# ChrisTho23/DrakeGPT

Hardware: NVIDIA B200
Metric: train_tokens_per_sec_TransformerLM_scaled (higher is better)
Workload: dtype bf16

## Files before the change

### drakegpt_b200/csrc/attn_tc.cu

```cuda
#include <cuda.h>

#include "common.cuh"
#include "ptx.cuh"

namespace dgpt {

using namespace ptx;

int make_tmap_bf16_2d(CUtensorMap* map, const void* base, int64_t inner, int64_t outer, int64_t ld, int box_outer);

static constexpr int HD = 64;
static constexpr int QT = 128;
static constexpr float kLog2e = 1.4426950408889634f;

struct AttnTcP {
  void *o, *dq, *dk, *dv;
  const void *o_in, *d_o;
  float* lse;
  int64_t o_rs, dq_rs, dk_rs, dv_rs, do_rs;
  int B, NH, T;
  float scale, inv_keep;
  uint32_t thr, site;
  uint64_t seed;
  const uint64_t* seed_dev;
};

__device__ __forceinline__ uint32_t pack_bf16(float a, float b) {
  __nv_bfloat162 v = __floats2bfloat162_rn(a, b);
  return *reinterpret_cast<uint32_t*>(&v);
}

__device__ __forceinline__ void store_row32_sw128(uint8_t* tile_base, int row, int c0, const float (&v)[32]) {
  uint8_t* blk = tile_base + (c0 >> 6) * 16384 + row * 128;
  const int chunk0 = (c0 & 63) >> 3;
#pragma unroll
  for (int j = 0; j < 4; ++j) {
    uint4 w;
    w.x = pack_bf16(v[8 * j], v[8 * j + 1]);
    w.y = pack_bf16(v[8 * j + 2], v[8 * j + 3]);
    w.z = pack_bf16(v[8 * j + 4], v[8 * j + 5]);
    w.w = pack_bf16(v[8 * j + 6], v[8 * j + 7]);
    *reinterpret_cast<uint4*>(blk + (((chunk0 + j) ^ (row & 7)) << 4)) = w;
  }
}

static constexpr int kFwd2Threads = 320;
static constexpr int kFwd2QK = 49152;
static constexpr int kFwd2Smem = 2 * kFwd2QK + 2 * 32768 + 256 + 1024;
static constexpr int kWHeavy = 5, kWLight = 2;

struct FwdSched {
  int nheavy, nlight;
  unsigned long long* probe;
};

__global__ void __launch_bounds__(kFwd2Threads, 1)
attn_fwd_tc2_kernel(const __grid_constant__ CUtensorMap map_q32, const __grid_constant__ CUtensorMap map_k,
                    const __grid_constant__ CUtensorMap map_v, AttnTcP p, FwdSched sc) {
  extern __shared__ uint8_t smem_raw[];
  uint8_t* smem = reinterpret_cast<uint8_t*>((reinterpret_cast<uintptr_t>(smem_raw) + 1023) & ~(uintptr_t)1023);
  uint8_t* sQK = smem;
  uint8_t* sV = smem + 2 * kFwd2QK;
  uint64_t* bars = reinterpret_cast<uint64_t*>(sV + 2 * 32768);
  uint64_t *qk_full = bars, *qk_empty = bars + 2, *v_full = bars + 4, *v_empty = bars + 6, *s_full = bars + 8,
           *p_full = bars + 10, *o_full = bars + 12, *slot_free = bars + 14;
  uint32_t* tmem_slot = reinterpret_cast<uint32_t*>(bars + 16);

  clock_probe_begin(sc.probe);
  const int warp = threadIdx.x >> 5, lane = threadIdx.x & 31;
  const int ntile = p.T / QT;

  const int G = gridDim.x, c = blockIdx.x;
  const int hq = sc.nheavy / G, hr = sc.nheavy % G;
  const int nh_c = hq + (c < hr ? 1 : 0);
  const int U = (kWHeavy * sc.nheavy + kWLight * sc.nlight + G - 1) / G;
  const int cap_hi = max(0, (U - kWHeavy * (hq + 1)) / kWLight), cap_lo = max(0, (U - kWHeavy * hq) / kWLight);
  const int cap_total = hr * cap_hi + (G - hr) * cap_lo;
  const int l_start = c < hr ? c * cap_hi : hr * cap_hi + (c - hr) * cap_lo;
  const int l0 = min(sc.nlight, l_start), l1 = min(sc.nlight, l_start + (c < hr ? cap_hi : cap_lo));
  const int n_extra = cap_total < sc.nlight ? (sc.nlight - cap_total - c + G - 1) / G : 0;
  const int n_items = nh_c + (l1 - l0) + max(0, n_extra);
  auto item = [&](int n, int& bh, int& qt) {
    if (n < nh_c) {
      const int hi = c + n * G;
      bh = hi; qt = ntile - 1;
    } else {
      const int m = n - nh_c;
      const int li = m < l1 - l0 ? l0 + m : cap_total + c + (m - (l1 - l0)) * G;
      bh = li; qt = 0;
    }
  };

  if (threadIdx.x == 0) {
    prefetch_tensormap(&map_q32);
    prefetch_tensormap(&map_k);
    prefetch_tensormap(&map_v);
    for (int g = 0; g < 2; ++g) {
      mbar_init(&qk_full[g], 1);
      mbar_init(&qk_empty[g], 1);
      mbar_init(&v_full[g], 1);
      mbar_init(&v_empty[g], 1);
      mbar_init(&s_full[g], 1);
      mbar_init(&p_full[g], 4);
      mbar_init(&o_full[g], 1);
      mbar_init(&slot_free[g], 4);
    }
    fence_barrier_init();
  }
  if (warp == 9) tmem_alloc<512>(tmem_slot);
  tc_fence_before();
  __syncthreads();
  tc_fence_after();
  const uint32_t tmem = *tmem_slot;
  pdl_grid_sync();

  if (warp == 8) {
    for (int n = 0; n < n_items; ++n) {
      const int g = n & 1, k = n >> 1;
      int bh, qt;
      item(n, bh, qt);
      const int nkv = qt + 1, b = bh / p.NH, h = bh % p.NH, row0 = b * p.T;
      uint8_t* q_s = sQK + g * kFwd2QK;
      uint8_t* v_s = sV + g * 32768;
      mbar_wait(&qk_empty[g], (k & 1) ^ 1);
      if (elect_one()) {
        mbar_expect_tx(&qk_full[g], 16384 * (1 + nkv));
        for (int qb = 0; qb < 4; ++qb)
          tma_load_2d(q_s + qb * 4096, &map_q32, &qk_full[g], h * HD, row0 + qt * QT + (g ? 3 - qb : qb) * 32);
        for (int j = 0; j < nkv; ++j) tma_load_2d(q_s + 16384 * (1 + j), &map_k, &qk_full[g], h * HD, row0 + j * QT);
      }
      __syncwarp();
      mbar_wait(&v_empty[g], (k & 1) ^ 1);
      if (elect_one()) {
        mbar_expect_tx(&v_full[g], 16384 * nkv);
        for (int kb = 0; kb < 2 * nkv; ++kb) tma_load_2d(v_s + kb * 8192, &map_v, &v_full[g], h * HD, row0 + kb * 64);
      }
      __syncwarp();
    }
  } else if (warp == 9) {
    constexpr uint32_t idesc_s = make_idesc_bf16(128, 128, 0, 0);
    constexpr uint32_t idesc_o = make_idesc_bf16(128, 64, 0, 1);
    int next_s = 0, next_pv = 0;
    while (next_pv < n_items) {
      bool progressed = false;
      if (next_s < n_items) {
        const int g = next_s & 1, k = next_s >> 1;
        if (mbar_test(&qk_full[g], k & 1) && mbar_test(&slot_free[g], (k & 1) ^ 1)) {
          tc_fence_after();
          int bh, qt;
          item(next_s, bh, qt);
          const int nkv = qt + 1;
          const uint64_t dq0 = make_smem_desc_sw128(smem_u32(sQK + g * kFwd2QK), 16, 1024);
          const uint64_t dk0 = make_smem_desc_sw128(smem_u32(sQK + g * kFwd2QK + 16384), 16, 1024);
          if (elect_one()) {
            for (int j = 0; j < nkv; ++j) {
#pragma unroll
              for (int kk = 0; kk < 4; ++kk)
                tc_mma_bf16(tmem + g * 256 + j * 128, dq0 + (uint64_t)(kk * 2), dk0 + (uint64_t)(j * 1024 + kk * 2), idesc_s, kk > 0);
            }
            tc_commit(&s_full[g]);
            tc_commit(&qk_empty[g]);
          }
          __syncwarp();
          ++next_s;
          progressed = true;
        }
      }
      if (next_pv < next_s) {
        const int g = next_pv & 1, k = next_pv >> 1;
        if (mbar_test(&p_full[g], k & 1) && mbar_test(&v_full[g], k & 1)) {
          tc_fence_after();
          int bh, qt;
          item(next_pv, bh, qt);
          const int nkv = qt + 1;
          const uint64_t dv0 = make_smem_desc_sw128(smem_u32(sV + g * 32768), 8192, 1024);
          if (elect_one()) {
            for (int kb = 0; kb < 2 * nkv; ++kb) {
#pragma unroll
              for (int kk = 0; kk < 4; ++kk)
                tc_mma_bf16_ts(tmem + g * 256 + nkv * 64, tmem + g * 256 + kb * 32 + kk * 8, dv0 + (uint64_t)(kb * 512 + kk * 128),
                               idesc_o, (kb | kk) > 0);
            }
            tc_commit(&o_full[g]);
            tc_commit(&v_empty[g]);
          }
          __syncwarp();
          ++next_pv;
          progressed = true;
        }
      }
      if (!progressed) __nanosleep(32);
    }
  } else {
    const int g = warp >> 2;
    const int quad = warp & 3;
    const int rblk = g ? 3 - quad : quad;
    const int row = rblk * 32 + lane;
    const uint32_t taddr = tmem + (uint32_t)(g * 256) + ((uint32_t)(quad * 32) << 16);
    uint64_t seed = p.seed;
    if (p.thr && p.seed_dev) seed += *p.seed_dev;
    const float sc2 = p.scale * kLog2e;
    for (int n = g; n < n_items; n += 2) {
      const int k = n >> 1;
      int bh, qt;
      item(n, bh, qt);
      const int nkv = qt + 1, b = bh / p.NH, h = bh % p.NH, row0 = b * p.T;
      const int qg = qt * QT + row;
      const int ncols = nkv * QT;
#define FTS(i) do { if (sc.probe && blockIdx.x == 0 && warp == 0 && lane == 0 && k < 3) sc.probe[4 + k * 8 + (i)] = (unsigned long long)clock64(); } while (0)
      FTS(0);
      mbar_wait(&s_full[g], k & 1);
      FTS(1);
      tc_fence_after();
      const int qg_max = qt * QT + rblk * 32 + 31, qg_min = qt * QT + rblk * 32;
      float mx = -INFINITY;
      for (int cc = 0; cc < ncols && cc <= qg_max; cc += 32) {
        uint32_t r[32];
        tmem_ld32(taddr + cc, r);
        tmem_ld_wait();
        if (cc + 31 <= qg_min) {
#pragma unroll
          for (int j = 0; j < 32; ++j) mx = fmaxf(mx, __uint_as_float(r[j]));
        } else {
#pragma unroll
          for (int j = 0; j < 32; ++j)
            if (cc + j <= qg) mx = fmaxf(mx, __uint_as_float(r[j]));
        }
      }
      FTS(2);
      const float msc = mx * sc2;
      float sum = 0.f;
      const uint64_t base = (((uint64_t)b * p.NH + h) * p.T + qg) * (uint64_t)p.T;
      for (int cc = 0; cc < ncols; cc += 32) {
        float e[32];
        if (cc > qg_max) {
#pragma unroll
          for (int j = 0; j < 32; ++j) e[j] = 0.f;
        } else {
          uint32_t r[32];
          tmem_ld32(taddr + cc, r);
          tmem_ld_wait();
          if (cc + 31 <= qg_min) {
#pragma unroll
            for (int j = 0; j < 32; ++j) {
              const float v = exp2f(__uint_as_float(r[j]) * sc2 - msc);
              sum += v;
              e[j] = v;
            }
          } else {
#pragma unroll
            for (int j = 0; j < 32; ++j) {
              const float v = (cc + j <= qg) ? exp2f(__uint_as_float(r[j]) * sc2 - msc) : 0.f;
              sum += v;
              e[j] = v;
            }
          }
          if (p.thr) {
            const DropGroup dg = dropout_group(seed, p.site, (base + cc) >> 5);
#pragma unroll
            for (int j = 0; j < 32; ++j)
              if (dropout_word(dg, j) < p.thr) e[j] = 0.f;
          }
        }
        uint32_t pk[16];
#pragma unroll
        for (int j = 0; j < 16; ++j) pk[j] = pack_bf16(e[2 * j], e[2 * j + 1]);
        tmem_st16(taddr + (cc >> 1), pk);
      }
      if (p.lse) p.lse[((int64_t)b * p.NH + h) * p.T + qg] = mx * p.scale + logf(sum);
      tmem_st_wait();
      tc_fence_before();
      __syncwarp();
      if (lane == 0) mbar_arrive(&p_full[g]);
      FTS(3);
      mbar_wait(&o_full[g], k & 1);
      FTS(4);
      tc_fence_after();
      const float oscale = p.inv_keep / sum;
      __nv_bfloat16* orow = reinterpret_cast<__nv_bfloat16*>(p.o) + (int64_t)(row0 + qg) * p.o_rs + h * HD;
#pragma unroll
      for (int cc = 0; cc < HD; cc += 32) {
        uint32_t r[32];
        tmem_ld32(taddr + nkv * 64 + cc, r);
        tmem_ld_wait();
#pragma unroll
        for (int j = 0; j < 4; ++j) {
          uint4 w;
          w.x = pack_bf16(__uint_as_float(r[8 * j]) * oscale, __uint_as_float(r[8 * j + 1]) * oscale);
          w.y = pack_bf16(__uint_as_float(r[8 * j + 2]) * oscale, __uint_as_float(r[8 * j + 3]) * oscale);
          w.z = pack_bf16(__uint_as_float(r[8 * j + 4]) * oscale, __uint_as_float(r[8 * j + 5]) * oscale);
          w.w = pack_bf16(__uint_as_float(r[8 * j + 6]) * oscale, __uint_as_float(r[8 * j + 7]) * oscale);
          *reinterpret_cast<uint4*>(orow + cc + 8 * j) = w;
        }
      }
      tc_fence_before();
      __syncwarp();
      if (lane == 0) mbar_arrive(&slot_free[g]);
      FTS(5);
    }
  }
  tc_fence_before();
  __syncthreads();
  if (warp == 9) {
    tc_fence_after();
    tmem_dealloc<512>(tmem);
  }
  clock_probe_end(sc.probe);
}

#ifdef DGPT_ATTN_TS
__device__ long long g_attn_ts[64];
#endif
static constexpr int kBwdThreads = 64 + 256;
static constexpr int kBwdSmem = 8 * 16384 + 2 * 32768 + 16384 + 2048 + 1024 + 128;

template <bool DIAG, bool DROP>
__device__ __forceinline__ void bwd_chunk_math(const AttnTcP& p, uint32_t lane_addr_st, uint32_t lane_addr_dp, int row, int k0,
                                               float sc, float lse2, float Dq, uint64_t seed, uint64_t base,
                                               float (&pd)[32], float (&ds)[32]) {
  uint32_t st[32], dp[32];
  tmem_ld32(lane_addr_st + k0, st);
  tmem_ld32(lane_addr_dp + k0, dp);
  tmem_ld_wait();
  DropGroup g = {0u, 0u};
  if (DROP) g = dropout_group(seed, p.site, (base + k0) >> 5);
#pragma unroll
  for (int t = 0; t < 32; ++t) {
    float pv = exp2f(__uint_as_float(st[t]) * sc - lse2);
    if (DIAG) pv = (k0 + t) <= row ? pv : 0.f;
    float dpv = __uint_as_float(dp[t]);
    float pdv = pv;
    if (DROP) {
      const bool keep = dropout_word(g, t) >= p.thr;
      dpv = keep ? dpv * p.inv_keep : 0.f;
      pdv = keep ? pv * p.inv_keep : 0.f;
    }
    pd[t] = pdv;
    ds[t] = pv * (dpv - Dq) * p.scale;
  }
}

template <bool DROP>
__global__ void __launch_bounds__(kBwdThreads, 1)
attn_bwd_tc_kernel(const __grid_constant__ CUtensorMap map_q, const __grid_constant__ CUtensorMap map_k,
                   const __grid_constant__ CUtensorMap map_v, const __grid_constant__ CUtensorMap map_do,
                   const __grid_constant__ CUtensorMap map_o, const __grid_constant__ CUtensorMap map_dq,
                   const __grid_constant__ CUtensorMap map_dk, const __grid_constant__ CUtensorMap map_dv, AttnTcP p) {
  extern __shared__ __align__(1024) uint8_t smem[];
  uint8_t* sQ = smem;
  uint8_t* sK = smem + 2 * 16384;
  uint8_t* sV = smem + 4 * 16384;
  uint8_t* sG = smem + 6 * 16384;
  uint8_t* sPd = smem + 8 * 16384;
  uint8_t* sDs = sPd + 32768;
  uint8_t* sSt = sDs + 32768;
  float* lse_s = reinterpret_cast<float*>(sSt + 16384);
  float* D_s = lse_s + 256;
  uint64_t* bars = reinterpret_cast<uint64_t*>(D_s + 256);
  uint64_t *ld_a = bars, *st_full = bars + 1, *ps_full = bars + 2, *drained = bars + 3, *acc_done = bars + 4;
  uint64_t *ld_b = bars + 5, *ld_c = bars + 6;
  uint64_t* acc_free = bars + 7;
  uint32_t* tmem_slot = reinterpret_cast<uint32_t*>(bars + 8);

  const int warp = threadIdx.x >> 5, lane = threadIdx.x & 31;
#ifdef DGPT_ATTN_TS
#define BTS(i) do { if (blockIdx.x == 0 && blockIdx.y == (gridDim.y / 2) && warp == 2 && lane == 0) g_attn_ts[i] = clock64(); } while (0)
#else
#define BTS(i) do { } while (0)
#endif
  BTS(0);
  const int h = blockIdx.x, b = blockIdx.y;
  const int ntile = p.T / QT;
  const int npair = ntile == 1 ? 1 : 3;
  const int row0 = b * p.T;

  if (threadIdx.x == 0) {
    prefetch_tensormap(&map_q);
    prefetch_tensormap(&map_k);
    prefetch_tensormap(&map_v);
    prefetch_tensormap(&map_do);
    prefetch_tensormap(&map_o);
    mbar_init(ld_a, 1);
    mbar_init(ld_b, 1);
    mbar_init(ld_c, 1);
    mbar_init(st_full, 1);
    mbar_init(ps_full, 8);
    mbar_init(drained, 8);
    mbar_init(acc_done, 1);
    mbar_init(acc_free, 1);
    fence_barrier_init();
  }
  if (warp == 0) {
    __syncwarp();
    pdl_grid_sync();
    if (elect_one()) {
      mbar_expect_tx(ld_a, 16384 * 5);
      tma_load_2d(sG, &map_do, ld_a, h * HD, row0);
      tma_load_2d(sPd, &map_o, ld_a, h * HD, row0);
      tma_load_2d(sQ, &map_q, ld_a, h * HD, row0);
      tma_load_2d(sK, &map_k, ld_a, h * HD, row0);
      tma_load_2d(sV, &map_v, ld_a, h * HD, row0);
      if (ntile > 1) {
        mbar_expect_tx(ld_b, 16384 * 3);
        tma_load_2d(sG + 16384, &map_do, ld_b, h * HD, row0 + QT);
        tma_load_2d(sSt, &map_o, ld_b, h * HD, row0 + QT);
        tma_load_2d(sQ + 16384, &map_q, ld_b, h * HD, row0 + QT);
        mbar_expect_tx(ld_c, 16384 * 2);
        tma_load_2d(sK + 16384, &map_k, ld_c, h * HD, row0 + QT);
        tma_load_2d(sV + 16384, &map_v, ld_c, h * HD, row0 + QT);
      }
    }
  }
  if (warp == 1) tmem_alloc<512>(tmem_slot);
  tc_fence_before();
  __syncthreads();
  tc_fence_after();
  const uint32_t tmem = *tmem_slot;
  constexpr uint32_t TM_ST = 0, TM_DP = 128, TM_DV = 256, TM_DK = 320, TM_DQ = 384;
  if (warp != 0) pdl_grid_sync();

  if (warp == 0) {
  } else if (warp == 1) {
    constexpr uint32_t id_kk = make_idesc_bf16(128, 128, 0, 0);
    constexpr uint32_t id_kmn = make_idesc_bf16(128, 64, 0, 1);
    constexpr uint32_t id_mnmn = make_idesc_bf16(128, 64, 1, 1);
    mbar_wait(ld_a, 0);
    tc_fence_after();
    const uint64_t kQ = make_smem_desc_sw128(smem_u32(sQ), 16, 1024), kK = make_smem_desc_sw128(smem_u32(sK), 16, 1024);
    const uint64_t kV = make_smem_desc_sw128(smem_u32(sV), 16, 1024), kG = make_smem_desc_sw128(smem_u32(sG), 16, 1024);
    const uint64_t kDs = make_smem_desc_sw128(smem_u32(sDs), 16, 1024);
    const uint64_t mQ = make_smem_desc_sw128(smem_u32(sQ), 8192, 1024), mK = make_smem_desc_sw128(smem_u32(sK), 8192, 1024);
    const uint64_t mG = make_smem_desc_sw128(smem_u32(sG), 8192, 1024);
    const uint64_t mPd = make_smem_desc_sw128(smem_u32(sPd), 16384, 1024), mDs = make_smem_desc_sw128(smem_u32(sDs), 16384, 1024);
    auto issue_s_dp = [&](int pr) {
      const int i = pr == 0 ? 0 : 1, j = pr == 2 ? 1 : 0;
      if (elect_one()) {
#pragma unroll
        for (int k = 0; k < 4; ++k)
          tc_mma_bf16(tmem + TM_ST, kQ + (uint64_t)(i * 1024 + k * 2), kK + (uint64_t)(j * 1024 + k * 2), id_kk, k > 0);
#pragma unroll
        for (int k = 0; k < 4; ++k)
          tc_mma_bf16(tmem + TM_DP, kG + (uint64_t)(i * 1024 + k * 2), kV + (uint64_t)(j * 1024 + k * 2), id_kk, k > 0);
        tc_commit(st_full);
      }
      __syncwarp();
    };
    issue_s_dp(0);
    for (int pr = 0; pr < npair; ++pr) {
      const int i = pr == 0 ? 0 : 1, j = pr == 2 ? 1 : 0;
      mbar_wait(ps_full, pr & 1);
      if (pr + 1 < npair) {
        mbar_wait(pr + 1 == 1 ? ld_b : ld_c, 0);
        tc_fence_after();
        issue_s_dp(pr + 1);
      }
      if (pr > 0) mbar_wait(drained, (pr - 1) & 1);
      tc_fence_after();
      const uint32_t acc_vk = (pr == 1) ? 1u : 0u;
      const uint32_t acc_q = (pr == 2) ? 1u : 0u;
      if (elect_one()) {
#pragma unroll
        for (int k = 0; k < 8; ++k)
          tc_mma_bf16(tmem + TM_DV, mPd + (uint64_t)(k * 128), mG + (uint64_t)(i * 1024 + k * 128), id_mnmn, acc_vk | (k > 0));
#pragma unroll
        for (int k = 0; k < 8; ++k)
          tc_mma_bf16(tmem + TM_DK, mDs + (uint64_t)(k * 128), mQ + (uint64_t)(i * 1024 + k * 128), id_mnmn, acc_vk | (k > 0));
#pragma unroll
        for (int k = 0; k < 8; ++k)
          tc_mma_bf16(tmem + TM_DQ, kDs + (uint64_t)((k >> 2) * 1024 + (k & 3) * 2), mK + (uint64_t)(j * 1024 + k * 128), id_kmn,
                      acc_q | (k > 0));
        tc_commit(acc_free);
        if (pr == npair - 1) tc_commit(acc_done);
      }
      __syncwarp();
    }
  } else {
    const int cw = warp - 2;
    const int quad = warp & 3;
    const int half = cw >> 2;
    const int rowl = quad * 32 + lane;
    const int ct = threadIdx.x - 64;
    const uint32_t lane_addr = tmem + ((uint32_t)(quad * 32) << 16);
    uint64_t seed = p.seed;
    if (DROP && p.seed_dev) seed += *p.seed_dev;
    if (ct < p.T) lse_s[ct] = p.lse[((int64_t)b * p.NH + h) * p.T + ct] * kLog2e;
    auto compute_D = [&](int tl, const uint8_t* o_tile) {
      if (ct < QT) {
        const int r = ct;
        const uint8_t* gr = sG + tl * 16384 + r * 128;
        const uint8_t* orow = o_tile + r * 128;
        float acc = 0.f;
#pragma unroll
        for (int c = 0; c < 8; ++c) {
          const int off = (c ^ (r & 7)) << 4;
          const uint4 g = *reinterpret_cast<const uint4*>(gr + off), o = *reinterpret_cast<const uint4*>(orow + off);
          const uint32_t gw[4] = {g.x, g.y, g.z, g.w}, ow[4] = {o.x, o.y, o.z, o.w};
#pragma unroll
          for (int t = 0; t < 4; ++t) {
            const float2 gf = __bfloat1622float2(*reinterpret_cast<const __nv_bfloat162*>(&gw[t]));
            const float2 of = __bfloat1622float2(*reinterpret_cast<const __nv_bfloat162*>(&ow[t]));
            acc = fmaf(gf.x, of.x, acc);
            acc = fmaf(gf.y, of.y, acc);
          }
        }
        D_s[tl * QT + r] = acc;
      }
      asm volatile("bar.sync 1, 256;" ::: "memory");
    };
    BTS(1);
    mbar_wait(ld_a, 0);
    BTS(2);
    compute_D(0, sPd);
    const float sc = p.scale * kLog2e;
    int n_stores = 0;

    auto drain = [&](uint32_t tm_col, const CUtensorMap* map, int tile) {
      uint32_t r[32];
      tmem_ld32(lane_addr + tm_col + half * 32, r);
      if (n_stores > 0) {
        if (ct == 0) bulk_wait_read<0>();
        asm volatile("bar.sync 1, 256;" ::: "memory");
      }
      tmem_ld_wait();
      uint8_t* rp = sSt + rowl * 128;
#pragma unroll
      for (int j = 0; j < 4; ++j) {
        uint4 w;
        w.x = pack_bf16(__uint_as_float(r[8 * j]), __uint_as_float(r[8 * j + 1]));
        w.y = pack_bf16(__uint_as_float(r[8 * j + 2]), __uint_as_float(r[8 * j + 3]));
        w.z = pack_bf16(__uint_as_float(r[8 * j + 4]), __uint_as_float(r[8 * j + 5]));
        w.w = pack_bf16(__uint_as_float(r[8 * j + 6]), __uint_as_float(r[8 * j + 7]));
        *reinterpret_cast<uint4*>(rp + (((half * 4 + j) ^ (rowl & 7)) << 4)) = w;
      }
      fence_proxy_async();
      asm volatile("bar.sync 1, 256;" ::: "memory");
      if (ct == 0) {
        tma_store_2d(map, sSt, h * HD, row0 + tile * QT);
        bulk_commit();
      }
      ++n_stores;
    };

    BTS(3);
    for (int pr = 0; pr < npair; ++pr) {
      const int i = pr == 0 ? 0 : 1, j = pr == 2 ? 1 : 0;
      if (pr == 1) {
        mbar_wait(ld_b, 0);
        compute_D(1, sSt);
      }
      BTS(4 + 4 * pr);
      mbar_wait(st_full, pr & 1);
      BTS(5 + 4 * pr);
      tc_fence_after();
      const int qi = i * QT + rowl;
      const float lse2 = lse_s[qi], Dq = D_s[qi];
      const uint64_t base = (((uint64_t)b * p.NH + h) * p.T + qi) * (uint64_t)p.T + (uint64_t)(j * QT);
      float pd[32], ds[32];
      if (i == j) bwd_chunk_math<true, DROP>(p, lane_addr + TM_ST, lane_addr + TM_DP, rowl, half * 64, sc, lse2, Dq, seed, base, pd, ds);
      else bwd_chunk_math<false, DROP>(p, lane_addr + TM_ST, lane_addr + TM_DP, rowl, half * 64, sc, lse2, Dq, seed, base, pd, ds);
      if (pr > 0) {
        mbar_wait(acc_free, (pr - 1) & 1);
        tc_fence_after();
        if (pr == 1) {
          drain(TM_DQ, &map_dq, 0);
        } else {
          drain(TM_DV, &map_dv, 0);
          drain(TM_DK, &map_dk, 0);
        }
        tc_fence_before();
        __syncwarp();
        if (lane == 0) mbar_arrive(drained);
      }
      BTS(6 + 4 * pr);
      store_row32_sw128(sPd, rowl, half * 64, pd);
      store_row32_sw128(sDs, rowl, half * 64, ds);
      if (i == j) bwd_chunk_math<true, DROP>(p, lane_addr + TM_ST, lane_addr + TM_DP, rowl, half * 64 + 32, sc, lse2, Dq, seed, base, pd, ds);
      else bwd_chunk_math<false, DROP>(p, lane_addr + TM_ST, lane_addr + TM_DP, rowl, half * 64 + 32, sc, lse2, Dq, seed, base, pd, ds);
      store_row32_sw128(sPd, rowl, half * 64 + 32, pd);
      store_row32_sw128(sDs, rowl, half * 64 + 32, ds);
      fence_proxy_async();
      tc_fence_before();
      __syncwarp();
      if (lane == 0) mbar_arrive(ps_full);
      BTS(7 + 4 * pr);
    }
    BTS(16);
    mbar_wait(acc_done, 0);
    BTS(17);
    tc_fence_after();
    const int last = ntile - 1;
    {
      if (n_stores > 0) {
        if (ct == 0) bulk_wait_read<0>();
        asm volatile("bar.sync 1, 256;" ::: "memory");
      }
      uint8_t* tiles[3] = {sPd, sDs, sSt};
      const uint32_t cols[3] = {TM_DV, TM_DK, TM_DQ};
#pragma unroll
      for (int q = 0; q < 3; ++q) {
        uint32_t r[32];
        tmem_ld32(lane_addr + cols[q] + half * 32, r);
        tmem_ld_wait();
        uint8_t* rp = tiles[q] + rowl * 128;
#pragma unroll
        for (int j = 0; j < 4; ++j) {
          uint4 w;
          w.x = pack_bf16(__uint_as_float(r[8 * j]), __uint_as_float(r[8 * j + 1]));
          w.y = pack_bf16(__uint_as_float(r[8 * j + 2]), __uint_as_float(r[8 * j + 3]));
          w.z = pack_bf16(__uint_as_float(r[8 * j + 4]), __uint_as_float(r[8 * j + 5]));
          w.w = pack_bf16(__uint_as_float(r[8 * j + 6]), __uint_as_float(r[8 * j + 7]));
          *reinterpret_cast<uint4*>(rp + (((half * 4 + j) ^ (rowl & 7)) << 4)) = w;
        }
      }
      fence_proxy_async();
      asm volatile("bar.sync 1, 256;" ::: "memory");
      if (ct == 0) {
        tma_store_2d(&map_dv, sPd, h * HD, row0 + last * QT);
        tma_store_2d(&map_dk, sDs, h * HD, row0 + last * QT);
        tma_store_2d(&map_dq, sSt, h * HD, row0 + last * QT);
        bulk_commit();
      }
    }
    if (ct == 0) bulk_wait<0>();
    BTS(18);
  }
  tc_fence_before();
  __syncthreads();
  if (warp == 1) {
    tc_fence_after();
    tmem_dealloc<512>(tmem);
  }
}

bool attn_tc_supported(const dgpt_attn_args* a) {
  if (a->dtype != DGPT_BF16 || a->H != HD || a->Tq != a->Tk) return false;
  if (a->Tk != 128 && a->Tk != 256) return false;
  const int64_t T = a->Tk;
  auto ok = [&](const void* ptr, int64_t bs, int64_t rs) {
    return ptr && ((uintptr_t)ptr & 15) == 0 && rs % 8 == 0 && bs == T * rs;
  };
  if (!ok(a->q, a->q_bs, a->q_rs) || !ok(a->k, a->k_bs, a->k_rs) || !ok(a->v, a->v_bs, a->v_rs) ||
      !ok(a->o, a->o_bs, a->o_rs))
    return false;
  if (a->d_o) {
    if (!ok(a->d_o, a->do_bs, a->do_rs) || !ok(a->dq, a->dq_bs, a->dq_rs) || !ok(a->dk, a->dk_bs, a->dk_rs) ||
        !ok(a->dv, a->dv_bs, a->dv_rs) || !a->lse)
      return false;
  }
  return true;
}

static AttnTcP make_tc_params(const dgpt_attn_args* a) {
  AttnTcP p;
  p.o = a->o; p.dq = a->dq; p.dk = a->dk; p.dv = a->dv; p.o_in = a->o; p.d_o = a->d_o; p.lse = a->lse;
  p.o_rs = a->o_rs; p.dq_rs = a->dq_rs; p.dk_rs = a->dk_rs; p.dv_rs = a->dv_rs; p.do_rs = a->do_rs;
  p.B = a->B; p.NH = a->NH; p.T = a->Tk;
  p.scale = a->scale; p.inv_keep = 1.f / (1.f - a->dropout_p);
  p.thr = dropout_threshold(a->dropout_p); p.site = a->site; p.seed = a->seed; p.seed_dev = a->seed_dev;
  return p;
}

int launch_attn_fwd_tc(const dgpt_attn_args* a, cudaStream_t st) {
  CUtensorMap mq, mk, mv;
  const int64_t rows = (int64_t)a->B * a->Tk, cols = (int64_t)a->NH * HD;
  int rc;
  if ((rc = make_tmap_bf16_2d(&mq, a->q, cols, rows, a->q_rs, 32))) return rc;
  if ((rc = make_tmap_bf16_2d(&mk, a->k, cols, rows, a->k_rs, QT))) return rc;
  if ((rc = make_tmap_bf16_2d(&mv, a->v, cols, rows, a->v_rs, 64))) return rc;
  AttnTcP p = make_tc_params(a);
  static bool attr = false;
  if (!attr) {
    cudaError_t e = cudaFuncSetAttribute(attn_fwd_tc2_kernel, cudaFuncAttributeMaxDynamicSharedMemorySize, kFwd2Smem);
    if (e != cudaSuccess) { set_error("attn_fwd_tc2: smem attribute: %s", cudaGetErrorString(e)); return DGPT_E_LAUNCH; }
    attr = true;
  }
  const int ntile = a->Tk / QT, bh = a->B * a->NH;
  FwdSched sc;
  sc.nheavy = ntile > 1 ? bh : 0;
  sc.nlight = bh;
  sc.probe = clock_probe_buffer();
  int sms = dgpt_sm_count();
  if (sms <= 0) sms = 148;
  const int grid = min(sms, sc.nheavy + sc.nlight);
  launch_pdl(attn_fwd_tc2_kernel, dim3(grid), dim3(kFwd2Threads), kFwd2Smem, st, mq, mk, mv, p, sc);
  return check_launch("attn_fwd_tc2");
}

int launch_attn_bwd_tc(const dgpt_attn_args* a, cudaStream_t st) {
  CUtensorMap mq, mk, mv, mg, mo, mdq, mdk, mdv;
  const int64_t rows = (int64_t)a->B * a->Tk, cols = (int64_t)a->NH * HD;
  int rc;
  if ((rc = make_tmap_bf16_2d(&mq, a->q, cols, rows, a->q_rs, QT))) return rc;
  if ((rc = make_tmap_bf16_2d(&mk, a->k, cols, rows, a->k_rs, QT))) return rc;
  if ((rc = make_tmap_bf16_2d(&mv, a->v, cols, rows, a->v_rs, QT))) return rc;
  if ((rc = make_tmap_bf16_2d(&mg, a->d_o, cols, rows, a->do_rs, QT))) return rc;
  if ((rc = make_tmap_bf16_2d(&mo, a->o, cols, rows, a->o_rs, QT))) return rc;
  if ((rc = make_tmap_bf16_2d(&mdq, a->dq, cols, rows, a->dq_rs, QT))) return rc;
  if ((rc = make_tmap_bf16_2d(&mdk, a->dk, cols, rows, a->dk_rs, QT))) return rc;
  if ((rc = make_tmap_bf16_2d(&mdv, a->dv, cols, rows, a->dv_rs, QT))) return rc;
  static bool attr = false;
  if (!attr) {
    cudaError_t e = cudaFuncSetAttribute(attn_bwd_tc_kernel<true>, cudaFuncAttributeMaxDynamicSharedMemorySize, kBwdSmem);
    if (e == cudaSuccess)
      e = cudaFuncSetAttribute(attn_bwd_tc_kernel<false>, cudaFuncAttributeMaxDynamicSharedMemorySize, kBwdSmem);
    if (e != cudaSuccess) { set_error("attn_bwd_tc: smem attribute: %s", cudaGetErrorString(e)); return DGPT_E_LAUNCH; }
    attr = true;
  }
  AttnTcP p = make_tc_params(a);
  dim3 grid(a->NH, a->B);
  if (p.thr) launch_pdl(attn_bwd_tc_kernel<true>, grid, dim3(kBwdThreads), kBwdSmem, st, mq, mk, mv, mg, mo, mdq, mdk, mdv, p);
  else launch_pdl(attn_bwd_tc_kernel<false>, grid, dim3(kBwdThreads), kBwdSmem, st, mq, mk, mv, mg, mo, mdq, mdk, mdv, p);
#ifdef DGPT_ATTN_TS
  {
    cudaStreamSynchronize(st);
    long long h[64];
    cudaMemcpyFromSymbol(h, g_attn_ts, sizeof(h));
    printf("attn bwd CTA: setup %lld | load wait %lld | D %lld |", h[1] - h[0], h[2] - h[1], h[3] - h[2]);
    for (int pr = 0; pr < 3; ++pr)
      printf(" pair%d: S/dP wait %lld, drains %lld, chunks %lld |", pr, h[5 + 4 * pr] - h[4 + 4 * pr], h[6 + 4 * pr] - h[5 + 4 * pr],
             h[7 + 4 * pr] - h[6 + 4 * pr]);
    printf(" acc wait %lld | final drains %lld | total %lld\n", h[17] - h[16], h[18] - h[17], h[18] - h[0]);
    fflush(stdout);
  }
#endif
  return check_launch("attn_bwd_tc");
}

}
```

Baseline: 7.864 million.

## Make attention backward kernel persistent with cross-item load and TMEM pipelining

Replaces the one-CTA-per-(batch,head) grid with a persistent grid of up to SM-count CTAs that loop over items. New mbarriers (a_free, tm_free, st_free) let the TMA warp prefetch the next item's Q/K/V/dO/O tiles while the current item finishes, and let the MMA warp start the next item's S/dP while the final dK/dV/dQ tiles are still being drained to global memory. The final drains are staged through freed Q/K/dO buffers, and the next item's LSE row is prefetched into a register. This hides per-CTA launch, setup and TMEM-allocation cost across items, at the price of much more complex barrier phase tracking and a risk of races or deadlock.

```diff
diff --git a/drakegpt_b200/csrc/attn_tc.cu b/drakegpt_b200/csrc/attn_tc.cu
--- a/drakegpt_b200/csrc/attn_tc.cu
+++ b/drakegpt_b200/csrc/attn_tc.cu
@@ -360,19 +360,19 @@
   uint64_t *ld_a = bars, *st_full = bars + 1, *ps_full = bars + 2, *drained = bars + 3, *acc_done = bars + 4;
   uint64_t *ld_b = bars + 5, *ld_c = bars + 6;
   uint64_t* acc_free = bars + 7;
-  uint32_t* tmem_slot = reinterpret_cast<uint32_t*>(bars + 8);
+  uint64_t *a_free = bars + 8, *tm_free = bars + 9, *st_free = bars + 10;
+  uint32_t* tmem_slot = reinterpret_cast<uint32_t*>(bars + 11);
 
   const int warp = threadIdx.x >> 5, lane = threadIdx.x & 31;
 #ifdef DGPT_ATTN_TS
-#define BTS(i) do { if (blockIdx.x == 0 && blockIdx.y == (gridDim.y / 2) && warp == 2 && lane == 0) g_attn_ts[i] = clock64(); } while (0)
+#define BTS(i) do { if (blockIdx.x == 0 && it < 3 && warp == 2 && lane == 0) g_attn_ts[it * 20 + (i)] = clock64(); } while (0)
+  if (blockIdx.x == 0 && warp == 2 && lane == 0) g_attn_ts[60] = clock64();
 #else
 #define BTS(i) do { } while (0)
 #endif
-  BTS(0);
-  const int h = blockIdx.x, b = blockIdx.y;
+  const int nitems = p.B * p.NH;
   const int ntile = p.T / QT;
   const int npair = ntile == 1 ? 1 : 3;
-  const int row0 = b * p.T;
 
   if (threadIdx.x == 0) {
     prefetch_tensormap(&map_q);
@@ -388,19 +388,30 @@
     mbar_init(drained, 8);
     mbar_init(acc_done, 1);
     mbar_init(acc_free, 1);
+    mbar_init(a_free, 1);
+    mbar_init(tm_free, 8);
+    mbar_init(st_free, 1);
     fence_barrier_init();
   }
-  if (warp == 0) {
-    __syncwarp();
-    pdl_grid_sync();
+
+  auto load_item = [&](int it, int item) {
+    const int b = item / p.NH, h = item % p.NH, row0 = b * p.T;
+    const uint32_t prev = (it - 1) & 1;
+    if (it > 0) mbar_wait(a_free, prev);
     if (elect_one()) {
       mbar_expect_tx(ld_a, 16384 * 5);
       tma_load_2d(sG, &map_do, ld_a, h * HD, row0);
-      tma_load_2d(sPd, &map_o, ld_a, h * HD, row0);
       tma_load_2d(sQ, &map_q, ld_a, h * HD, row0);
       tma_load_2d(sK, &map_k, ld_a, h * HD, row0);
       tma_load_2d(sV, &map_v, ld_a, h * HD, row0);
-      if (ntile > 1) {
+    }
+    __syncwarp();
+    if (it > 0) mbar_wait(acc_done, prev);
+    if (elect_one()) tma_load_2d(sPd, &map_o, ld_a, h * HD, row0);
+    __syncwarp();
+    if (ntile > 1) {
+      if (it > 0) mbar_wait(st_free, prev);
+      if (elect_one()) {
         mbar_expect_tx(ld_b, 16384 * 3);
         tma_load_2d(sG + 16384, &map_do, ld_b, h * HD, row0 + QT);
         tma_load_2d(sSt, &map_o, ld_b, h * HD, row0 + QT);
@@ -409,7 +420,13 @@
         tma_load_2d(sK + 16384, &map_k, ld_c, h * HD, row0 + QT);
         tma_load_2d(sV + 16384, &map_v, ld_c, h * HD, row0 + QT);
       }
-    }
+      __syncwarp();
+    }
+  };
+  if (warp == 0) {
+    __syncwarp();
+    pdl_grid_sync();
+    load_item(0, blockIdx.x);
   }
   if (warp == 1) tmem_alloc<512>(tmem_slot);
   tc_fence_before();
@@ -420,12 +437,11 @@
   if (warp != 0) pdl_grid_sync();
 
   if (warp == 0) {
+    for (int it = 1, item = blockIdx.x + gridDim.x; item < nitems; ++it, item += gridDim.x) load_item(it, item);
   } else if (warp == 1) {
     constexpr uint32_t id_kk = make_idesc_bf16(128, 128, 0, 0);
     constexpr uint32_t id_kmn = make_idesc_bf16(128, 64, 0, 1);
     constexpr uint32_t id_mnmn = make_idesc_bf16(128, 64, 1, 1);
-    mbar_wait(ld_a, 0);
-    tc_fence_after();
     const uint64_t kQ = make_smem_desc_sw128(smem_u32(sQ), 16, 1024), kK = make_smem_desc_sw128(smem_u32(sK), 16, 1024);
     const uint64_t kV = make_smem_desc_sw128(smem_u32(sV), 16, 1024), kG = make_smem_desc_sw128(smem_u32(sG), 16, 1024);
     const uint64_t kDs = make_smem_desc_sw128(smem_u32(sDs), 16, 1024);
@@ -445,35 +461,49 @@
       }
       __syncwarp();
     };
-    issue_s_dp(0);
-    for (int pr = 0; pr < npair; ++pr) {
-      const int i = pr == 0 ? 0 : 1, j = pr == 2 ? 1 : 0;
-      mbar_wait(ps_full, pr & 1);
-      if (pr + 1 < npair) {
-        mbar_wait(pr + 1 == 1 ? ld_b : ld_c, 0);
+    uint32_t ph_ps = 0, ph_dr = 0;
+    auto mma_item = [&](int it) {
+      const uint32_t ph = it & 1;
+      mbar_wait(ld_a, ph);
+      tc_fence_after();
+      issue_s_dp(0);
+      for (int pr = 0; pr < npair; ++pr) {
+        mbar_wait(ps_full, ph_ps);
+        ph_ps ^= 1;
+        if (pr + 1 < npair) {
+          mbar_wait(pr + 1 == 1 ? ld_b : ld_c, ph);
+          tc_fence_after();
+          issue_s_dp(pr + 1);
+        }
+        if (pr > 0) {
+          mbar_wait(drained, ph_dr);
+          ph_dr ^= 1;
+        } else if (it > 0) {
+          mbar_wait(tm_free, ph ^ 1);
+        }
         tc_fence_after();
-        issue_s_dp(pr + 1);
-      }
-      if (pr > 0) mbar_wait(drained, (pr - 1) & 1);
-      tc_fence_after();
-      const uint32_t acc_vk = (pr == 1) ? 1u : 0u;
-      const uint32_t acc_q = (pr == 2) ? 1u : 0u;
-      if (elect_one()) {
-#pragma unroll
-        for (int k = 0; k < 8; ++k)
-          tc_mma_bf16(tmem + TM_DV, mPd + (uint64_t)(k * 128), mG + (uint64_t)(i * 1024 + k * 128), id_mnmn, acc_vk | (k > 0));
-#pragma unroll
-        for (int k = 0; k < 8; ++k)
-          tc_mma_bf16(tmem + TM_DK, mDs + (uint64_t)(k * 128), mQ + (uint64_t)(i * 1024 + k * 128), id_mnmn, acc_vk | (k > 0));
-#pragma unroll
-        for (int k = 0; k < 8; ++k)
-          tc_mma_bf16(tmem + TM_DQ, kDs + (uint64_t)((k >> 2) * 1024 + (k & 3) * 2), mK + (uint64_t)(j * 1024 + k * 128), id_kmn,
-                      acc_q | (k > 0));
-        tc_commit(acc_free);
-        if (pr == npair - 1) tc_commit(acc_done);
-      }
-      __syncwarp();
-    }
+        const int i = pr == 0 ? 0 : 1, j = pr == 2 ? 1 : 0;
+        const uint32_t acc_vk = (pr == 1) ? 1u : 0u;
+        const uint32_t acc_q = (pr == 2) ? 1u : 0u;
+        if (elect_one()) {
+#pragma unroll
+          for (int k = 0; k < 8; ++k)
+            tc_mma_bf16(tmem + TM_DV, mPd + (uint64_t)(k * 128), mG + (uint64_t)(i * 1024 + k * 128), id_mnmn, acc_vk | (k > 0));
+#pragma unroll
+          for (int k = 0; k < 8; ++k)
+            tc_mma_bf16(tmem + TM_DK, mDs + (uint64_t)(k * 128), mQ + (uint64_t)(i * 1024 + k * 128), id_mnmn, acc_vk | (k > 0));
+#pragma unroll
+          for (int k = 0; k < 8; ++k)
+            tc_mma_bf16(tmem + TM_DQ, kDs + (uint64_t)((k >> 2) * 1024 + (k & 3) * 2), mK + (uint64_t)(j * 1024 + k * 128), id_kmn,
+                        acc_q | (k > 0));
+          tc_commit(acc_free);
+          if (pr == (npair > 1 ? 1 : 0)) tc_commit(a_free);
+          if (pr == npair - 1) tc_commit(acc_done);
+        }
+        __syncwarp();
+      }
+    };
+    for (int it = 0, item = blockIdx.x; item < nitems; ++it, item += gridDim.x) mma_item(it);
   } else {
     const int cw = warp - 2;
     const int quad = warp & 3;
@@ -483,7 +513,6 @@
     const uint32_t lane_addr = tmem + ((uint32_t)(quad * 32) << 16);
     uint64_t seed = p.seed;
     if (DROP && p.seed_dev) seed += *p.seed_dev;
-    if (ct < p.T) lse_s[ct] = p.lse[((int64_t)b * p.NH + h) * p.T + ct] * kLog2e;
     auto compute_D = [&](int tl, const uint8_t* o_tile) {
       if (ct < QT) {
         const int r = ct;
@@ -507,101 +536,24 @@
       }
       asm volatile("bar.sync 1, 256;" ::: "memory");
     };
-    BTS(1);
-    mbar_wait(ld_a, 0);
-    BTS(2);
-    compute_D(0, sPd);
     const float sc = p.scale * kLog2e;
     int n_stores = 0;
-
-    auto drain = [&](uint32_t tm_col, const CUtensorMap* map, int tile) {
-      uint32_t r[32];
-      tmem_ld32(lane_addr + tm_col + half * 32, r);
-      if (n_stores > 0) {
-        if (ct == 0) bulk_wait_read<0>();
-        asm volatile("bar.sync 1, 256;" ::: "memory");
-      }
-      tmem_ld_wait();
-      uint8_t* rp = sSt + rowl * 128;
-#pragma unroll
-      for (int j = 0; j < 4; ++j) {
-        uint4 w;
-        w.x = pack_bf16(__uint_as_float(r[8 * j]), __uint_as_float(r[8 * j + 1]));
-        w.y = pack_bf16(__uint_as_float(r[8 * j + 2]), __uint_as_float(r[8 * j + 3]));
-        w.z = pack_bf16(__uint_as_float(r[8 * j + 4]), __uint_as_float(r[8 * j + 5]));
-        w.w = pack_bf16(__uint_as_float(r[8 * j + 6]), __uint_as_float(r[8 * j + 7]));
-        *reinterpret_cast<uint4*>(rp + (((half * 4 + j) ^ (rowl & 7)) << 4)) = w;
-      }
-      fence_proxy_async();
-      asm volatile("bar.sync 1, 256;" ::: "memory");
-      if (ct == 0) {
-        tma_store_2d(map, sSt, h * HD, row0 + tile * QT);
-        bulk_commit();
-      }
-      ++n_stores;
-    };
-
-    BTS(3);
-    for (int pr = 0; pr < npair; ++pr) {
-      const int i = pr == 0 ? 0 : 1, j = pr == 2 ? 1 : 0;
-      if (pr == 1) {
-        mbar_wait(ld_b, 0);
-        compute_D(1, sSt);
-      }
-      BTS(4 + 4 * pr);
-      mbar_wait(st_full, pr & 1);
-      BTS(5 + 4 * pr);
-      tc_fence_after();
-      const int qi = i * QT + rowl;
-      const float lse2 = lse_s[qi], Dq = D_s[qi];
-      const uint64_t base = (((uint64_t)b * p.NH + h) * p.T + qi) * (uint64_t)p.T + (uint64_t)(j * QT);
-      float pd[32], ds[32];
-      if (i == j) bwd_chunk_math<true, DROP>(p, lane_addr + TM_ST, lane_addr + TM_DP, rowl, half * 64, sc, lse2, Dq, seed, base, pd, ds);
-      else bwd_chunk_math<false, DROP>(p, lane_addr + TM_ST, lane_addr + TM_DP, rowl, half * 64, sc, lse2, Dq, seed, base, pd, ds);
-      if (pr > 0) {
-        mbar_wait(acc_free, (pr - 1) & 1);
-        tc_fence_after();
-        if (pr == 1) {
-          drain(TM_DQ, &map_dq, 0);
-        } else {
-          drain(TM_DV, &map_dv, 0);
-          drain(TM_DK, &map_dk, 0);
-        }
-        tc_fence_before();
-        __syncwarp();
-        if (lane == 0) mbar_arrive(drained);
-      }
-      BTS(6 + 4 * pr);
-      store_row32_sw128(sPd, rowl, half * 64, pd);
-      store_row32_sw128(sDs, rowl, half * 64, ds);
-      if (i == j) bwd_chunk_math<true, DROP>(p, lane_addr + TM_ST, lane_addr + TM_DP, rowl, half * 64 + 32, sc, lse2, Dq, seed, base, pd, ds);
-      else bwd_chunk_math<false, DROP>(p, lane_addr + TM_ST, lane_addr + TM_DP, rowl, half * 64 + 32, sc, lse2, Dq, seed, base, pd, ds);
-      store_row32_sw128(sPd, rowl, half * 64 + 32, pd);
-      store_row32_sw128(sDs, rowl, half * 64 + 32, ds);
-      fence_proxy_async();
-      tc_fence_before();
-      __syncwarp();
-      if (lane == 0) mbar_arrive(ps_full);
-      BTS(7 + 4 * pr);
-    }
-    BTS(16);
-    mbar_wait(acc_done, 0);
-    BTS(17);
-    tc_fence_after();
-    const int last = ntile - 1;
-    {
-      if (n_stores > 0) {
-        if (ct == 0) bulk_wait_read<0>();
-        asm volatile("bar.sync 1, 256;" ::: "memory");
-      }
-      uint8_t* tiles[3] = {sPd, sDs, sSt};
-      const uint32_t cols[3] = {TM_DV, TM_DK, TM_DQ};
-#pragma unroll
-      for (int q = 0; q < 3; ++q) {
+    uint32_t ph_st = 0, ph_af = 0;
+    float lse_r = ct < p.T ? p.lse[(int64_t)blockIdx.x * p.T + ct] : 0.f;
+
+    auto compute_item = [&](int it, int item) {
+      const int b = item / p.NH, h = item % p.NH, row0 = b * p.T;
+      const uint32_t ph = it & 1;
+
+      auto drain = [&](uint32_t tm_col, const CUtensorMap* map, int tile) {
         uint32_t r[32];
-        tmem_ld32(lane_addr + cols[q] + half * 32, r);
+        tmem_ld32(lane_addr + tm_col + half * 32, r);
+        if (n_stores > 0) {
+          if (ct == 0) bulk_wait_read<0>();
+          asm volatile("bar.sync 1, 256;" ::: "memory");
+        }
         tmem_ld_wait();
-        uint8_t* rp = tiles[q] + rowl * 128;
+        uint8_t* rp = sSt + rowl * 128;
 #pragma unroll
         for (int j = 0; j < 4; ++j) {
           uint4 w;
@@ -611,18 +563,119 @@
           w.w = pack_bf16(__uint_as_float(r[8 * j + 6]), __uint_as_float(r[8 * j + 7]));
           *reinterpret_cast<uint4*>(rp + (((half * 4 + j) ^ (rowl & 7)) << 4)) = w;
         }
-      }
-      fence_proxy_async();
-      asm volatile("bar.sync 1, 256;" ::: "memory");
-      if (ct == 0) {
-        tma_store_2d(&map_dv, sPd, h * HD, row0 + last * QT);
-        tma_store_2d(&map_dk, sDs, h * HD, row0 + last * QT);
-        tma_store_2d(&map_dq, sSt, h * HD, row0 + last * QT);
-        bulk_commit();
-      }
-    }
+        fence_proxy_async();
+        asm volatile("bar.sync 1, 256;" ::: "memory");
+        if (ct == 0) {
+          tma_store_2d(map, sSt, h * HD, row0 + tile * QT);
+          bulk_commit();
+        }
+        ++n_stores;
+      };
+
+      BTS(0);
+      if (ct < p.T) lse_s[ct] = lse_r * kLog2e;
+      BTS(1);
+      mbar_wait(ld_a, ph);
+      BTS(2);
+      compute_D(0, sPd);
+      if (ntile > 1 && it > 0 && ct == 0) {
+        bulk_wait_read<0>();
+        mbar_arrive(st_free);
+      }
+
+      BTS(3);
+      for (int pr = 0; pr < npair; ++pr) {
+        const int i = pr == 0 ? 0 : 1, j = pr == 2 ? 1 : 0;
+        if (pr == 1) {
+          mbar_wait(ld_b, ph);
+          compute_D(1, sSt);
+        }
+        BTS(4 + 4 * pr);
+        mbar_wait(st_full, ph_st);
+        ph_st ^= 1;
+        BTS(5 + 4 * pr);
+        tc_fence_after();
+        const int qi = i * QT + rowl;
+        const float lse2 = lse_s[qi], Dq = D_s[qi];
+        const uint64_t base = (((uint64_t)b * p.NH + h) * p.T + qi) * (uint64_t)p.T + (uint64_t)(j * QT);
+        float pd[32], ds[32];
+        if (i == j) bwd_chunk_math<true, DROP>(p, lane_addr + TM_ST, lane_addr + TM_DP, rowl, half * 64, sc, lse2, Dq, seed, base, pd, ds);
+        else bwd_chunk_math<false, DROP>(p, lane_addr + TM_ST, lane_addr + TM_DP, rowl, half * 64, sc, lse2, Dq, seed, base, pd, ds);
+        if (pr > 0) {
+          mbar_wait(acc_free, ph_af);
+          ph_af ^= 1;
+          tc_fence_after();
+          if (pr == 1) {
+            drain(TM_DQ, &map_dq, 0);
+          } else {
+            drain(TM_DV, &map_dv, 0);
+            drain(TM_DK, &map_dk, 0);
+          }
+          tc_fence_before();
+          __syncwarp();
+          if (lane == 0) mbar_arrive(drained);
+        }
+        BTS(6 + 4 * pr);
+        store_row32_sw128(sPd, rowl, half * 64, pd);
+        store_row32_sw128(sDs, rowl, half * 64, ds);
+        if (i == j) bwd_chunk_math<true, DROP>(p, lane_addr + TM_ST, lane_addr + TM_DP, rowl, half * 64 + 32, sc, lse2, Dq, seed, base, pd, ds);
+        else bwd_chunk_math<false, DROP>(p, lane_addr + TM_ST, lane_addr + TM_DP, rowl, half * 64 + 32, sc, lse2, Dq, seed, base, pd, ds);
+        store_row32_sw128(sPd, rowl, half * 64 + 32, pd);
+        store_row32_sw128(sDs, rowl, half * 64 + 32, ds);
+        fence_proxy_async();
+        tc_fence_before();
+        __syncwarp();
+        if (lane == 0) mbar_arrive(ps_full);
+        BTS(7 + 4 * pr);
+      }
+      BTS(16);
+      const int next = item + gridDim.x;
+      if (next < nitems && ct < p.T) lse_r = p.lse[(int64_t)next * p.T + ct];
+      mbar_wait(acc_done, ph);
+      ph_af ^= 1;
+      BTS(17);
+      tc_fence_after();
+      const int last = ntile - 1;
+      {
+        if (n_stores > 0) {
+          if (ct == 0) bulk_wait_read<0>();
+          asm volatile("bar.sync 1, 256;" ::: "memory");
+        }
+        uint8_t* tiles[3] = {sG + 16384, sQ + 16384, sK + 16384};
+        const uint32_t cols[3] = {TM_DV, TM_DK, TM_DQ};
+#pragma unroll
+        for (int q = 0; q < 3; ++q) {
+          uint32_t r[32];
+          tmem_ld32(lane_addr + cols[q] + half * 32, r);
+          tmem_ld_wait();
+          uint8_t* rp = tiles[q] + rowl * 128;
+#pragma unroll
+          for (int j = 0; j < 4; ++j) {
+            uint4 w;
+            w.x = pack_bf16(__uint_as_float(r[8 * j]), __uint_as_float(r[8 * j + 1]));
+            w.y = pack_bf16(__uint_as_float(r[8 * j + 2]), __uint_as_float(r[8 * j + 3]));
+            w.z = pack_bf16(__uint_as_float(r[8 * j + 4]), __uint_as_float(r[8 * j + 5]));
+            w.w = pack_bf16(__uint_as_float(r[8 * j + 6]), __uint_as_float(r[8 * j + 7]));
+            *reinterpret_cast<uint4*>(rp + (((half * 4 + j) ^ (rowl & 7)) << 4)) = w;
+          }
+        }
+        tc_fence_before();
+        __syncwarp();
+        if (lane == 0) mbar_arrive(tm_free);
+        fence_proxy_async();
+        asm volatile("bar.sync 1, 256;" ::: "memory");
+        if (ct == 0) {
+          tma_store_2d(&map_dv, tiles[0], h * HD, row0 + last * QT);
+          tma_store_2d(&map_dk, tiles[1], h * HD, row0 + last * QT);
+          tma_store_2d(&map_dq, tiles[2], h * HD, row0 + last * QT);
+          bulk_commit();
+        }
+        ++n_stores;
+      }
+      BTS(18);
+    };
+    for (int it = 0, item = blockIdx.x; item < nitems; ++it, item += gridDim.x) compute_item(it, item);
     if (ct == 0) bulk_wait<0>();
-    BTS(18);
   }
   tc_fence_before();
   __syncthreads();
@@ -631,6 +684,7 @@
     tmem_dealloc<512>(tmem);
   }
 }
+#undef BTS
 
 bool attn_tc_supported(const dgpt_attn_args* a) {
   if (a->dtype != DGPT_BF16 || a->H != HD || a->Tq != a->Tk) return false;
@@ -707,19 +761,27 @@
     attr = true;
   }
   AttnTcP p = make_tc_params(a);
-  dim3 grid(a->NH, a->B);
-  if (p.thr) launch_pdl(attn_bwd_tc_kernel<true>, grid, dim3(kBwdThreads), kBwdSmem, st, mq, mk, mv, mg, mo, mdq, mdk, mdv, p);
-  else launch_pdl(attn_bwd_tc_kernel<false>, grid, dim3(kBwdThreads), kBwdSmem, st, mq, mk, mv, mg, mo, mdq, mdk, mdv, p);
+  int sms = dgpt_sm_count();
+  if (sms <= 0) sms = 148;
+  const int nitems = a->B * a->NH;
+  const int grid = min(sms, nitems);
+  if (p.thr) launch_pdl(attn_bwd_tc_kernel<true>, dim3(grid), dim3(kBwdThreads), kBwdSmem, st, mq, mk, mv, mg, mo, mdq, mdk, mdv, p);
+  else launch_pdl(attn_bwd_tc_kernel<false>, dim3(grid), dim3(kBwdThreads), kBwdSmem, st, mq, mk, mv, mg, mo, mdq, mdk, mdv, p);
 #ifdef DGPT_ATTN_TS
   {
     cudaStreamSynchronize(st);
     long long h[64];
     cudaMemcpyFromSymbol(h, g_attn_ts, sizeof(h));
-    printf("attn bwd CTA: setup %lld | load wait %lld | D %lld |", h[1] - h[0], h[2] - h[1], h[3] - h[2]);
-    for (int pr = 0; pr < 3; ++pr)
-      printf(" pair%d: S/dP wait %lld, drains %lld, chunks %lld |", pr, h[5 + 4 * pr] - h[4 + 4 * pr], h[6 + 4 * pr] - h[5 + 4 * pr],
-             h[7 + 4 * pr] - h[6 + 4 * pr]);
-    printf(" acc wait %lld | final drains %lld | total %lld\n", h[17] - h[16], h[18] - h[17], h[18] - h[0]);
+    const int npair = a->Tk == 128 ? 1 : 3, n0 = min(3, (nitems + grid - 1) / grid);
+    printf("attn bwd CTA 0 (%d items): setup %lld\n", (nitems + grid - 1) / grid, h[0] - h[60]);
+    for (int n = 0; n < n0; ++n) {
+      const long long* t = h + 20 * n;
+      printf("  item %d at +%lld: lse %lld | load wait %lld | D %lld |", n, t[0] - h[60], t[1] - t[0], t[2] - t[1], t[3] - t[2]);
+      for (int pr = 0; pr < npair; ++pr)
+        printf(" pair%d: S/dP wait %lld, drains %lld, chunks %lld |", pr, t[5 + 4 * pr] - t[4 + 4 * pr], t[6 + 4 * pr] - t[5 + 4 * pr],
+               t[7 + 4 * pr] - t[6 + 4 * pr]);
+      printf(" acc wait %lld | final drains %lld | item %lld\n", t[17] - t[16], t[18] - t[17], t[18] - t[0]);
+    }
     fflush(stdout);
   }
 #endif
```

New measurement: 7.939 million, median of 6. Within noise of the previous version (+1.0%).
